# GLAD-RUC/DistEGNN

Hardware: NVIDIA H100
Metric: graph_steps_per_sec (higher is better)
Workload: dtype f32

## Files before the change

distegnn_b200/csrc/tc16.cuh:

```cuda
#pragma once
#include <cuda_fp16.h>

#include <type_traits>

#include "common.cuh"
#include "tile_mma.cuh"

namespace degnn {
namespace tc16 {

constexpr float RANGE = 3.0e4f;
__device__ __forceinline__ void split_pair(f32x2 x, uint32_t& hi, uint32_t& lo) {
    float x0, x1, l0, l1;
    upk2(x, x0, x1);
    const __half2 h = __floats2half2_rn(x0, x1);
    hi = *reinterpret_cast<const uint32_t*>(&h);
    const float2 hf = __half22float2(h);
    upk2(sub2(x, pk2(hf.x, hf.y)), l0, l1);
    const __half2 l = __floats2half2_rn(l0, l1);
    lo = *reinterpret_cast<const uint32_t*>(&l);
}

template <int NTHREADS>
__device__ __forceinline__ void stage_weight(__half* hi, __half* lo, const float* __restrict__ wt_kmajor, int n_off,
                                             int n_total, int tid, float scale = 1.0f) {
    static_assert((H * H) % NTHREADS == 0, "thread count must divide the matrix");
    constexpr int R = H * H / NTHREADS;
    const uint32_t lbo_h = (uint32_t)(n_total / 8) * 64u;
    float w[R];
#pragma unroll
    for (int r = 0; r < R; ++r) w[r] = __ldg(wt_kmajor + tid + r * NTHREADS);
#pragma unroll
    for (int r = 0; r < R; ++r) {
        const int i = tid + r * NTHREADS;
        const int k = i >> 6, n = (i & 63) + n_off;
        const float ws = w[r] * scale;
        const __half h = __float2half_rn(ws);
        const uint32_t o = (uint32_t)(k >> 3) * lbo_h + (uint32_t)(n >> 3) * 64u + (uint32_t)(n & 7) * 8u + (k & 7);
        hi[o] = h;
        lo[o] = __float2half_rn(ws - __half2float(h));
    }
}
__host__ __device__ constexpr uint32_t lbo_bytes(int n_total) { return (uint32_t)(n_total / 8) * 128u; }

template <uint32_t LBO>
__device__ __forceinline__ void mma_f16x3(uint32_t d, uint32_t a_hi, uint32_t a_lo, uint64_t b_hi, uint64_t b_lo,
                                          int nchunks, bool accumulate, int mb0, int nmb) {
    constexpr uint64_t B_KSTEP = (2 * LBO) >> 4, A_KSTEP = (2 * tmma::TM_COLGROUP_BYTES) >> 4, B_NCHUNK = (8 * 128) >> 4;
#pragma unroll 1
    for (int mb = mb0; mb < mb0 + nmb; ++mb) {
        const uint64_t ahi = tmma::make_desc(tmma::tm_addr_rc(64u * mb, a_hi), tmma::TM_COLGROUP_BYTES, 128);
        const uint64_t alo = tmma::make_desc(tmma::tm_addr_rc(64u * mb, a_lo), tmma::TM_COLGROUP_BYTES, 128);
#pragma unroll 1
        for (int nc = 0; nc < nchunks; ++nc) {
            float acc[32];
            if (accumulate) {
                tmma::frag_load(acc, d + 64u * nc, mb);
            } else {
#pragma unroll
                for (int i = 0; i < 32; ++i) acc[i] = 0.f;
            }
            const uint64_t bh = b_hi + nc * B_NCHUNK, bl = b_lo + nc * B_NCHUNK;
            tmma::wgmma_fence();
#pragma unroll
            for (int ks = 0; ks < 4; ++ks)
                tmma::wgmma_f16_m64n64k16(acc, alo + ks * A_KSTEP, bh + ks * B_KSTEP, (accumulate || ks > 0) ? 1u : 0u);
#pragma unroll
            for (int ks = 0; ks < 4; ++ks) tmma::wgmma_f16_m64n64k16(acc, ahi + ks * A_KSTEP, bl + ks * B_KSTEP, 1u);
#pragma unroll
            for (int ks = 0; ks < 4; ++ks) tmma::wgmma_f16_m64n64k16(acc, ahi + ks * A_KSTEP, bh + ks * B_KSTEP, 1u);
            tmma::wgmma_commit();
            tmma::wgmma_wait_all();
            tmma::frag_store(acc, d + 64u * nc, mb);
        }
    }
}

template <uint32_t LBO, bool ACCUMULATE = false>
__device__ __forceinline__ void mma_f16x3_rA(float (&d)[32], const uint32_t (&a_hi)[16], const uint32_t (&a_lo)[16],
                                             uint64_t b_hi, uint64_t b_lo) {
    constexpr uint64_t B_KSTEP = (2 * LBO) >> 4;
    auto mma = [&](auto acc, const uint32_t (&a)[16], int ks, uint64_t b) {
        tmma::wgmma_f16_m64n64k16_rA<decltype(acc)::value>(d, a[4 * ks], a[4 * ks + 1], a[4 * ks + 2], a[4 * ks + 3],
                                                            b + ks * B_KSTEP);
    };
    tmma::wgmma_fence();
    mma(std::integral_constant<bool, ACCUMULATE>{}, a_lo, 0, b_hi);
#pragma unroll
    for (int ks = 1; ks < 4; ++ks) mma(std::true_type{}, a_lo, ks, b_hi);
#pragma unroll
    for (int ks = 0; ks < 4; ++ks) mma(std::true_type{}, a_hi, ks, b_lo);
#pragma unroll
    for (int ks = 0; ks < 4; ++ks) mma(std::true_type{}, a_hi, ks, b_hi);
    tmma::wgmma_commit();
}
__device__ __forceinline__ void mma_f16x3_rA_wait(float (&d)[32], uint32_t (&a_hi)[16], uint32_t (&a_lo)[16]) {
    tmma::wgmma_wait_all();
#pragma unroll
    for (int i = 0; i < 32; ++i) tmma::wgmma_keep(d[i]);
#pragma unroll
    for (int i = 0; i < 16; ++i) {
        tmma::wgmma_keep(a_hi[i]);
        tmma::wgmma_keep(a_lo[i]);
    }
}

__device__ __forceinline__ bool row_overflow(__half2 mx) {
    return fmaxf(__low2float(mx), __high2float(mx)) > RANGE;
}
__device__ __forceinline__ void range_scale(float rowmax, float& s, float& inv_s) {
    const uint32_t eb = (__float_as_uint(rowmax) >> 23) & 0xffu;
    const uint32_t sb = eb > 141u ? 268u - eb : 127u;
    s = __uint_as_float((sb < 1u ? 1u : sb) << 23);
    inv_s = 1.0f / s;
}

constexpr std::false_type kFast{};
constexpr std::true_type kSafe{};
template <bool SCALED>
__device__ __forceinline__ void split16p(const f32x2 (&v)[8], float s, uint32_t (&hi)[8], uint32_t (&lo)[8],
                                         __half2& mx) {
#pragma unroll
    for (int j = 0; j < 8; ++j) {
        split_pair(SCALED ? mul2(v[j], bc2(s)) : v[j], hi[j], lo[j]);
        mx = __hmax2(mx, __habs2(*reinterpret_cast<const __half2*>(&hi[j])));
    }
}

}
}
```

distegnn_b200/csrc/tile_mma.cuh:

```cuda
#pragma once
#include <cuda_runtime.h>
#include <stdint.h>

namespace degnn {

extern __shared__ __align__(1024) uint8_t degnn_dyn_smem[];

namespace tmma {

constexpr uint32_t TM_COLGROUP_BYTES = 2048;
__host__ __device__ constexpr int tm_bytes(int ncols) { return ncols * 128 * 4; }

__device__ __forceinline__ uint32_t smem_u32(const void* p) {
    return (uint32_t)__cvta_generic_to_shared(p);
}

__device__ __forceinline__ uint32_t tm_addr_rc(uint32_t row, uint32_t col) {
    return smem_u32(degnn_dyn_smem) + (col >> 2) * TM_COLGROUP_BYTES + row * 16u + (col & 3u) * 4u;
}
__device__ __forceinline__ uint32_t tm_addr(uint32_t taddr) {
    return tm_addr_rc((taddr >> 16) + (threadIdx.x & 31u), taddr & 0xffffu);
}

__device__ __forceinline__ uint64_t make_desc(uint32_t smem_addr, uint32_t lbo, uint32_t sbo) {
    return (uint64_t)((smem_addr >> 4) & 0x3FFF) | ((uint64_t)((lbo >> 4) & 0x3FFF) << 16) |
           ((uint64_t)((sbo >> 4) & 0x3FFF) << 32);
}
__device__ __forceinline__ uint64_t make_b_desc(uint32_t smem_addr, uint32_t lbo, uint32_t sbo) {
    return make_desc(smem_addr, lbo, sbo);
}

__device__ __forceinline__ void fence_proxy_async_smem() { asm volatile("fence.proxy.async.shared::cta;" ::: "memory"); }
__device__ __forceinline__ void tm_st_fence() { fence_proxy_async_smem(); }

__device__ __forceinline__ void tm_st4(uint32_t taddr, const uint32_t (&r)[4]) {
    asm volatile("st.shared.v4.b32 [%0], {%1,%2,%3,%4};" ::"r"(tm_addr(taddr)), "r"(r[0]), "r"(r[1]), "r"(r[2]), "r"(r[3])
                 : "memory");
}
__device__ __forceinline__ void tm_ld4(uint32_t taddr, uint32_t* r) {
    asm volatile("ld.shared.v4.b32 {%0,%1,%2,%3}, [%4];" : "=r"(r[0]), "=r"(r[1]), "=r"(r[2]), "=r"(r[3]) : "r"(tm_addr(taddr))
                 : "memory");
}
__device__ __forceinline__ void tm_st8(uint32_t taddr, const uint32_t (&r)[8]) {
    tm_st4(taddr, *reinterpret_cast<const uint32_t(*)[4]>(&r[0]));
    tm_st4(taddr + 4, *reinterpret_cast<const uint32_t(*)[4]>(&r[4]));
}
__device__ __forceinline__ void tm_st16(uint32_t taddr, const uint32_t (&r)[16]) {
#pragma unroll
    for (int i = 0; i < 4; ++i) tm_st4(taddr + 4 * i, *reinterpret_cast<const uint32_t(*)[4]>(&r[4 * i]));
}
__device__ __forceinline__ void tm_ld8(uint32_t taddr, uint32_t (&r)[8]) {
    tm_ld4(taddr, &r[0]);
    tm_ld4(taddr + 4, &r[4]);
}
__device__ __forceinline__ void tm_ld16(uint32_t taddr, uint32_t (&r)[16]) {
#pragma unroll
    for (int i = 0; i < 4; ++i) tm_ld4(taddr + 4 * i, &r[4 * i]);
}
__device__ __forceinline__ void prefetch_l1(const void* p) { asm volatile("prefetch.global.L1 [%0];" ::"l"(p)); }
__device__ __forceinline__ void prefetch_l2(const void* p) { asm volatile("prefetch.global.L2 [%0];" ::"l"(p)); }

__device__ __forceinline__ void wgmma_fence() { asm volatile("wgmma.fence.sync.aligned;" ::: "memory"); }
__device__ __forceinline__ void wgmma_commit() { asm volatile("wgmma.commit_group.sync.aligned;" ::: "memory"); }
__device__ __forceinline__ void wgmma_wait_all() { asm volatile("wgmma.wait_group.sync.aligned 0;" ::: "memory"); }
__device__ __forceinline__ void wgmma_f16_m64n64k16(float (&d)[32], uint64_t a_desc, uint64_t b_desc, uint32_t accumulate) {
    asm volatile(
        "{\n\t"
        ".reg .pred p;\n\t"
        "setp.ne.b32 p, %34, 0;\n\t"
        "wgmma.mma_async.sync.aligned.m64n64k16.f32.f16.f16 "
        "{%0,%1,%2,%3,%4,%5,%6,%7,%8,%9,%10,%11,%12,%13,%14,%15,%16,%17,%18,%19,%20,%21,%22,%23,%24,%25,%26,%27,%28,%29,%30,%31},"
        " %32, %33, p, 1, 1, 0, 0;\n\t"
        "}\n"
        : "+f"(d[0]), "+f"(d[1]), "+f"(d[2]), "+f"(d[3]), "+f"(d[4]), "+f"(d[5]), "+f"(d[6]), "+f"(d[7]), "+f"(d[8]),
          "+f"(d[9]), "+f"(d[10]), "+f"(d[11]), "+f"(d[12]), "+f"(d[13]), "+f"(d[14]), "+f"(d[15]), "+f"(d[16]),
          "+f"(d[17]), "+f"(d[18]), "+f"(d[19]), "+f"(d[20]), "+f"(d[21]), "+f"(d[22]), "+f"(d[23]), "+f"(d[24]),
          "+f"(d[25]), "+f"(d[26]), "+f"(d[27]), "+f"(d[28]), "+f"(d[29]), "+f"(d[30]), "+f"(d[31])
        : "l"(a_desc), "l"(b_desc), "r"(accumulate)
        : "memory");
}
#define DEGNN_WGMMA_RA_D(c)                                                                                             \
    c(d[0]), c(d[1]), c(d[2]), c(d[3]), c(d[4]), c(d[5]), c(d[6]), c(d[7]), c(d[8]), c(d[9]), c(d[10]), c(d[11]),      \
        c(d[12]), c(d[13]), c(d[14]), c(d[15]), c(d[16]), c(d[17]), c(d[18]), c(d[19]), c(d[20]), c(d[21]), c(d[22]),  \
        c(d[23]), c(d[24]), c(d[25]), c(d[26]), c(d[27]), c(d[28]), c(d[29]), c(d[30]), c(d[31])
#define DEGNN_WGMMA_RA_ASM(scale_d)                                                                                     \
    "wgmma.mma_async.sync.aligned.m64n64k16.f32.f16.f16 "                                                               \
    "{%0,%1,%2,%3,%4,%5,%6,%7,%8,%9,%10,%11,%12,%13,%14,%15,%16,%17,%18,%19,%20,%21,%22,%23,%24,%25,%26,%27,%28,%29,%30," \
    "%31}, {%32,%33,%34,%35}, %36, " scale_d ", 1, 1, 0;\n"
template <bool ACCUMULATE>
__device__ __forceinline__ void wgmma_f16_m64n64k16_rA(float (&d)[32], uint32_t a0, uint32_t a1, uint32_t a2, uint32_t a3,
                                                       uint64_t b_desc) {
    if (ACCUMULATE)
        asm volatile(DEGNN_WGMMA_RA_ASM("1") : DEGNN_WGMMA_RA_D("+f")
                     : "r"(a0), "r"(a1), "r"(a2), "r"(a3), "l"(b_desc) : "memory");
    else
        asm volatile(DEGNN_WGMMA_RA_ASM("0") : DEGNN_WGMMA_RA_D("=f")
                     : "r"(a0), "r"(a1), "r"(a2), "r"(a3), "l"(b_desc) : "memory");
}
#undef DEGNN_WGMMA_RA_D
#undef DEGNN_WGMMA_RA_ASM
__device__ __forceinline__ void wgmma_keep(float& r) { asm volatile("" : "+f"(r)::"memory"); }
__device__ __forceinline__ void wgmma_keep(uint32_t& r) { asm volatile("" : "+r"(r)::"memory"); }
__device__ __forceinline__ void frag_rows(int mb, uint32_t& r0, uint32_t& q) {
    const uint32_t w = (threadIdx.x >> 5) & 3u, l = threadIdx.x & 31u;
    r0 = 64u * (uint32_t)mb + 16u * w + (l >> 2);
    q = l & 3u;
}
__device__ __forceinline__ void frag_store(const float (&d)[32], uint32_t col, int mb) {
    uint32_t r0, q;
    frag_rows(mb, r0, q);
#pragma unroll
    for (int j = 0; j < 8; ++j) {
        const uint32_t c = col + 8u * j + 2u * q;
        const uint32_t a0 = tm_addr_rc(r0, c), a1 = tm_addr_rc(r0 + 8u, c);
        asm volatile("st.shared.v2.f32 [%0], {%1,%2};" ::"r"(a0), "f"(d[4 * j]), "f"(d[4 * j + 1]) : "memory");
        asm volatile("st.shared.v2.f32 [%0], {%1,%2};" ::"r"(a1), "f"(d[4 * j + 2]), "f"(d[4 * j + 3]) : "memory");
    }
}
__device__ __forceinline__ void frag_load(float (&d)[32], uint32_t col, int mb) {
    uint32_t r0, q;
    frag_rows(mb, r0, q);
#pragma unroll
    for (int j = 0; j < 8; ++j) {
        const uint32_t c = col + 8u * j + 2u * q;
        asm volatile("ld.shared.v2.f32 {%0,%1}, [%2];" : "=f"(d[4 * j]), "=f"(d[4 * j + 1]) : "r"(tm_addr_rc(r0, c)) : "memory");
        asm volatile("ld.shared.v2.f32 {%0,%1}, [%2];" : "=f"(d[4 * j + 2]), "=f"(d[4 * j + 3]) : "r"(tm_addr_rc(r0 + 8u, c))
                     : "memory");
    }
}

__device__ __forceinline__ void mbar_init(uint64_t* bar, uint32_t count) {
    asm volatile("mbarrier.init.shared::cta.b64 [%0], %1;" ::"r"(smem_u32(bar)), "r"(count) : "memory");
}
__device__ __forceinline__ void fence_mbar_init() { asm volatile("fence.mbarrier_init.release.cluster;" ::: "memory"); }
__device__ __forceinline__ void mbar_expect_tx(uint64_t* bar, uint32_t bytes) {
    asm volatile("mbarrier.arrive.expect_tx.shared::cta.b64 _, [%0], %1;" ::"r"(smem_u32(bar)), "r"(bytes) : "memory");
}
__device__ __forceinline__ void mbar_wait(uint64_t* bar, uint32_t parity) {
    asm volatile(
        "{\n\t"
        ".reg .pred p;\n\t"
        "WAIT_LOOP:\n\t"
        "mbarrier.try_wait.parity.shared::cta.b64 p, [%0], %1;\n\t"
        "@p bra WAIT_DONE;\n\t"
        "bra WAIT_LOOP;\n\t"
        "WAIT_DONE:\n\t"
        "}\n" ::"r"(smem_u32(bar)),
        "r"(parity)
        : "memory");
}

__device__ __forceinline__ void bulk_g2s(void* smem_dst, const void* gsrc, uint32_t bytes, uint64_t* bar) {
    asm volatile("cp.async.bulk.shared::cluster.global.mbarrier::complete_tx::bytes [%0], [%1], %2, [%3];" ::"r"(
                     smem_u32(smem_dst)),
                 "l"(gsrc), "r"(bytes), "r"(smem_u32(bar))
                 : "memory");
}

__device__ __forceinline__ void cp_async16(void* smem_dst, const void* gsrc) {
    asm volatile("cp.async.cg.shared.global [%0], [%1], 16;" ::"r"(smem_u32(smem_dst)), "l"(gsrc) : "memory");
}
__device__ __forceinline__ void cp_async8(void* smem_dst, const void* gsrc) {
    asm volatile("cp.async.ca.shared.global [%0], [%1], 8;" ::"r"(smem_u32(smem_dst)), "l"(gsrc) : "memory");
}
__device__ __forceinline__ void cp_async4(void* smem_dst, const void* gsrc) {
    asm volatile("cp.async.ca.shared.global [%0], [%1], 4;" ::"r"(smem_u32(smem_dst)), "l"(gsrc) : "memory");
}
__device__ __forceinline__ void cp_async_commit() { asm volatile("cp.async.commit_group;" ::: "memory"); }
__device__ __forceinline__ void cp_async_wait_all() { asm volatile("cp.async.wait_group 0;" ::: "memory"); }
__device__ __forceinline__ void red_add_v2(float* gdst, float a, float b) {
    asm volatile("red.global.add.v2.f32 [%0], {%1, %2};" ::"l"(gdst), "f"(a), "f"(b) : "memory");
}

__device__ __forceinline__ void named_bar(uint32_t id, uint32_t nthreads) {
    asm volatile("bar.sync %0, %1;" ::"r"(id), "r"(nthreads) : "memory");
}

}
}
```

distegnn_b200/csrc/virtual_layer_tc16.cu:

```cuda
#include "common.cuh"
#include "det.cuh"
#include "tc16.cuh"
#include "tile_mma.cuh"

namespace degnn {

struct VirtT16Args {
    int64_t N;
    int B, C;
    unsigned flags;
    const int32_t* batch;
    const float* x4;
    const float* Hn;
    const float* Xv;
    const float* G;
    const float* w1r;
    const float* w2; const float* b2;
    const float* wxv; const float* bxv; const float* w3xv;
    const float* wx; const float* bx; const float* w3x;
    float* agg_v;
    float* trans_v;
    float* vsum;
    float* slots;
    int chunk_shift;
};

constexpr int VW_WG = 4;
constexpr int VW_THREADS = 128 * VW_WG, VW_WARPS = VW_THREADS / 32;
constexpr int VW_TILE = 64;
constexpr int VW_ROW = 72;
constexpr int VW_W = 64 * 64;
constexpr uint32_t VW_LBO = 1024;
__host__ __device__ constexpr int vw_smem_floats(int C) {
    return 6 * VW_W / 2 + 6 * H + VW_WARPS * 16 * VW_ROW + VW_WG * VW_TILE * 6 + VW_WG * C * VW_ROW + VW_WARPS * C * H
           + VW_WARPS * 4 * C;
}
__host__ __device__ constexpr int vw_smem_bytes(int C) { return vw_smem_floats(C) * 4; }
using tc16::kFast;
using tc16::kSafe;

static_assert(VW_TILE == DET_VTILE, "det.cuh sizes the slots from the tile");
template <bool DET>
__global__ void __launch_bounds__(VW_THREADS, 1) virtual_layer_t16_kernel(const VirtT16Args a) {
    using namespace tmma;
    const int C = a.C;
    __half* W2hi = reinterpret_cast<__half*>(degnn_dyn_smem);
    __half* W2lo = W2hi + VW_W;
    __half* Wxvhi = W2lo + VW_W;
    __half* Wxvlo = Wxvhi + VW_W;
    __half* Wxhi = Wxvlo + VW_W;
    __half* Wxlo = Wxhi + VW_W;
    float* w1rs = reinterpret_cast<float*>(Wxlo + VW_W);
    float* b2s = w1rs + H;
    float* bxvs = b2s + H;
    float* w3xvs = bxvs + H;
    float* bxs = w3xvs + H;
    float* w3xs = bxs + H;
    float* stage_all = w3xs + H;
    float* dX_all = stage_all + VW_WARPS * 16 * VW_ROW;
    float* phi_all = dX_all + VW_WG * VW_TILE * 4;
    float* gs_all = phi_all + VW_WG * VW_TILE * 2;
    float* accH_all = gs_all + VW_WG * C * VW_ROW;
    float* accX_all = accH_all + VW_WARPS * C * H;

    const int tid = threadIdx.x;
    const int lane = tid & 31;
    const int warp = tid >> 5;
    const int wg = warp >> 2;
    const int w = warp & 3;
    const int t = tid & 127;
    const int g = lane >> 2, q = lane & 3;
    const int K = 4 + 3 * C + H * C;
    const bool need_feat = !(a.flags & DISTEGNN_FLAG_LAST);
    const int TN = VW_TILE / C;
    const bool warp_local = (16 % C) == 0;

    tc16::stage_weight<VW_THREADS>(W2hi, W2lo, a.w2, 0, 64, tid, SILU_T_IN);
    tc16::stage_weight<VW_THREADS>(Wxvhi, Wxvlo, a.wxv, 0, 64, tid);
    tc16::stage_weight<VW_THREADS>(Wxhi, Wxlo, a.wx, 0, 64, tid);
    if (tid < H) {
        w1rs[tid] = a.w1r[tid];
        b2s[tid] = a.b2[tid] * SILU_T_IN;
        bxvs[tid] = a.bxv[tid] * SILU_T_IN;
        w3xvs[tid] = a.w3xv[tid] * SILU_T_OUT;
        bxs[tid] = a.bx[tid] * SILU_T_IN;
        w3xs[tid] = a.w3x[tid] * SILU_T_OUT;
    }
    for (int i = tid; i < VW_WARPS * (C * H + 4 * C); i += VW_THREADS) accH_all[i] = 0.f;
    fence_proxy_async_smem();
    __syncthreads();

    const uint64_t bW0 = make_b_desc(smem_u32(W2hi), VW_LBO, 128);
    auto bW = [&](int k) { return bW0 + (uint64_t)(k * (VW_W * 2 / 16)); };
    float* tile_s = stage_all + wg * VW_TILE * VW_ROW;
    float* dXs = dX_all + wg * VW_TILE * 4;
    float* phis = phi_all + wg * VW_TILE * 2;
    float* gs = gs_all + wg * C * VW_ROW;
    float* accH = accH_all + warp * C * H;
    float* accX = accX_all + warp * 4 * C;
    float* accH_g = accH_all + 4 * wg * C * H;
    float* accX_g = accX_all + 4 * wg * 4 * C;
    const uint32_t bar_id = 1 + wg;
    int cur_graph = -1;

    auto flush = [&](int gr) {
        if (gr < 0) return;
        float* dst = a.vsum + (size_t)gr * K;
        if (need_feat)
            for (int i = t; i < C * H; i += 128) {
                float s = 0.f;
#pragma unroll
                for (int k = 0; k < 4; ++k) {
                    s += accH_g[k * C * H + i];
                    accH_g[k * C * H + i] = 0.f;
                }
                atomicAdd(dst + 4 + 3 * C + i, s * SILU_T_OUT);
            }
        if (t < 3 * C) {
            float s = 0.f;
#pragma unroll
            for (int k = 0; k < 4; ++k) {
                s += accX_g[k * 4 * C + t];
                accX_g[k * 4 * C + t] = 0.f;
            }
            atomicAdd(dst + 4 + t, s);
        }
    };

    const int num_tiles = (int)((a.N + TN - 1) / TN);
    const int stride = (int)gridDim.x * VW_WG;
    const int CH = 1 << a.chunk_shift;
    auto next_tile = [&](int tl) {
        if constexpr (DET) return (tl + 1) % CH != 0 ? tl + 1 : tl + 1 + (stride - 1) * CH;
        else return tl + stride;
    };
    float* accG = accH_all + 4 * wg * C * H;
    float* accXG = accX_all + 4 * wg * 4 * C;
    int curM = -1, curX = -1, cont = -1;
    auto det_dst = [&](int gr, int tl) {
        return gr == cont ? a.slots + (size_t)(tl >> a.chunk_shift) * K : a.vsum + (size_t)gr * K;
    };
    auto det_flush_m = [&](int tl) {
        for (int c = t >> 5; c < C; c += 4) {
            f32x2* acc = reinterpret_cast<f32x2*>(accG + c * H + 2 * (t & 31));
            if (curM >= 0) {
                float* dst = det_dst(curM, tl) + 4 + 3 * C + c * H + 2 * (t & 31);
                upk2(mul2(*acc, bc2(SILU_T_OUT)), dst[0], dst[1]);
            }
            *acc = 0ull;
        }
    };
    auto det_flush_x = [&](int tl) {
        if (t < 3 * C) {
            if (curX >= 0) det_dst(curX, tl)[4 + t] = accXG[t];
            accXG[t] = 0.f;
        }
    };
    const int ra = 16 * w + g, rb = ra + 8;
    const float* colp = tile_s + 2 * lane;

    for (int tile = DET ? ((int)blockIdx.x * VW_WG + wg) * CH : (int)blockIdx.x * VW_WG + wg; tile < num_tiles;
         tile = next_tile(tile)) {
        const int64_t n0 = (int64_t)tile * TN;
        if (DET && tile % CH == 0)
            cont = (n0 > 0 && __ldg(a.batch + n0 - 1) == __ldg(a.batch + n0)) ? __ldg(a.batch + n0) : -1;
        const int nvalid = (int)min((int64_t)TN, a.N - n0);
        const int rows = nvalid * C;
        {
            const int64_t nn0 = (int64_t)next_tile(tile) * TN;
            const int nnv = (int)min((int64_t)TN, a.N - nn0);
            for (int i = t; i < 2 * nnv; i += 128) prefetch_l1(a.Hn + (size_t)nn0 * H + 32 * i);
            if (nnv > 0) {
                if (t < (nnv * 16 + 127) / 128) prefetch_l1(a.x4 + (size_t)nn0 * 4 + 32 * t);
                if (t == 127) prefetch_l1(a.batch + nn0);
                if (t == 126) prefetch_l1(a.batch + nn0 + nnv - 1);
            }
        }
        const int g_first = __ldg(a.batch + n0), g_last = __ldg(a.batch + n0 + nvalid - 1);
        const bool single = (g_first == g_last);
        if (single && g_first != cur_graph) {
            named_bar(bar_id, 128);
            if constexpr (!DET) flush(cur_graph);
            cur_graph = g_first;
            for (int i = t; i < C * (H / 4); i += 128) {
                const int c = i / (H / 4), q4 = i - c * (H / 4);
                *reinterpret_cast<float4*>(gs + c * VW_ROW + 4 * q4) = ldg4(a.G + ((size_t)g_first * C + c) * H + 4 * q4);
            }
            named_bar(bar_id, 128);
        }

        const bool va = ra < rows, vb = rb < rows;
        const float* pa;
        const float* pb;
        const float* ga;
        const float* gb;
        float vra, vrb;
        {
            auto row_geo = [&](int r, bool v, const float*& hrow, const float*& grow) {
                const int nl = v ? r / C : 0, ch = v ? r - nl * C : 0;
                const size_t node = (size_t)(n0 + nl);
                const int gr = single ? g_first : __ldg(a.batch + node);
                const float4 xi = ldg4(a.x4 + node * 4);
                const float* Xg = a.Xv + (size_t)gr * 3 * C;
                const float dx = __ldg(Xg + ch) - xi.x, dy = __ldg(Xg + C + ch) - xi.y, dz = __ldg(Xg + 2 * C + ch) - xi.z;
                if (q == 0) *reinterpret_cast<float4*>(dXs + 4 * r) = make_float4(dx, dy, dz, 0.f);
                hrow = a.Hn + node * H + 2 * q;
                grow = (gr == cur_graph ? (const float*)(gs + ch * VW_ROW) : a.G + ((size_t)gr * C + ch) * H) + 2 * q;
                return sqrtf(dx * dx + dy * dy + dz * dz);
            };
            vra = row_geo(ra, va, pa, ga);
            vrb = row_geo(rb, vb, pb, gb);
        }
        auto pre = [&](int j, const float* hrow, const float* grow, float vr) {
            const f32x2 hh = __ldg(reinterpret_cast<const f32x2*>(hrow + 8 * j));
            const f32x2 gg = *reinterpret_cast<const f32x2*>(grow + 8 * j);
            return fma2(bc2(vr), *reinterpret_cast<const f32x2*>(w1rs + 8 * j + 2 * q), add2(hh, gg));
        };
        uint32_t ahi[16], alo[16];
        float inv1a = 1.0f, inv1b = 1.0f;
        {
            __half2 mx = __floats2half2_rn(0.f, 0.f);
            float qmax = 0.f;
#pragma unroll
            for (int j = 0; j < 8; ++j) {
                f32x2 xa = pre(j, pa, ga, vra), xb = pre(j, pb, gb, vrb);
                silu4p<false>(xa, xb, qmax);
                if (!va) xa = 0ull;
                if (!vb) xb = 0ull;
                tc16::split_pair(xa, ahi[2 * j], alo[2 * j]);
                tc16::split_pair(xb, ahi[2 * j + 1], alo[2 * j + 1]);
                mx = __hmax2(mx, __hmax2(*reinterpret_cast<const __half2*>(&ahi[2 * j]),
                                         *reinterpret_cast<const __half2*>(&ahi[2 * j + 1])));
            }
            if (__any_sync(FULL, tc16::row_overflow(mx) || silu_q_overflow(qmax))) {
                float fa = 0.f, fb = 0.f, sa, sb;
#pragma unroll 1
                for (int j = 0; j < 8; ++j) {
                    f32x2 xa = pre(j, pa, ga, vra), xb = pre(j, pb, gb, vrb);
                    silu4p<true>(xa, xb, qmax);
                    float v0, v1;
                    upk2(xa, v0, v1);
                    if (va) fa = fmaxf(fa, fmaxf(v0, v1));
                    upk2(xb, v0, v1);
                    if (vb) fb = fmaxf(fb, fmaxf(v0, v1));
                }
                fa = fmaxf(fa, __shfl_xor_sync(FULL, fa, 1));
                fa = fmaxf(fa, __shfl_xor_sync(FULL, fa, 2));
                fb = fmaxf(fb, __shfl_xor_sync(FULL, fb, 1));
                fb = fmaxf(fb, __shfl_xor_sync(FULL, fb, 2));
                tc16::range_scale(fa, sa, inv1a);
                tc16::range_scale(fb, sb, inv1b);
#pragma unroll
                for (int j = 0; j < 8; ++j) {
                    f32x2 xa = pre(j, pa, ga, vra), xb = pre(j, pb, gb, vrb);
                    silu4p<true>(xa, xb, qmax);
                    if (!va) xa = 0ull;
                    if (!vb) xb = 0ull;
                    tc16::split_pair(mul2(xa, bc2(sa)), ahi[2 * j], alo[2 * j]);
                    tc16::split_pair(mul2(xb, bc2(sb)), ahi[2 * j + 1], alo[2 * j + 1]);
                }
            }
        }

        float d[32];
        tc16::mma_f16x3_rA<VW_LBO>(d, ahi, alo, bW(0), bW(1));
        tc16::mma_f16x3_rA_wait(d, ahi, alo);

        float inv2a = 1.0f, inv2b = 1.0f, s2a = 1.0f, s2b = 1.0f;
        auto m_pair = [&](int j, f32x2& ma, f32x2& mb) {
            const f32x2 bb = *reinterpret_cast<const f32x2*>(b2s + 8 * j + 2 * q);
            ma = fma2(pk2(d[4 * j + 0], d[4 * j + 1]), bc2(inv1a), bb);
            mb = fma2(pk2(d[4 * j + 2], d[4 * j + 3]), bc2(inv1b), bb);
        };
        auto store_m = [&](int j, f32x2 ma, f32x2 mb) {
            *reinterpret_cast<f32x2*>(tile_s + ra * VW_ROW + 8 * j + 2 * q) = ma;
            *reinterpret_cast<f32x2*>(tile_s + rb * VW_ROW + 8 * j + 2 * q) = mb;
        };
        {
            __half2 mx = __floats2half2_rn(0.f, 0.f);
            float qmax = 0.f;
#pragma unroll
            for (int j = 0; j < 8; ++j) {
                f32x2 ma, mb;
                m_pair(j, ma, mb);
                silu4t<false>(ma, mb, qmax);
                store_m(j, ma, mb);
                tc16::split_pair(ma, ahi[2 * j], alo[2 * j]);
                tc16::split_pair(mb, ahi[2 * j + 1], alo[2 * j + 1]);
                mx = __hmin2(mx, __hmin2(*reinterpret_cast<const __half2*>(&ahi[2 * j]),
                                         *reinterpret_cast<const __half2*>(&ahi[2 * j + 1])));
            }
            if (__any_sync(FULL, fminf(__low2float(mx), __high2float(mx)) < -tc16::RANGE || silu_q_overflow(qmax))) {
                float fa = 0.f, fb = 0.f;
#pragma unroll
                for (int j = 0; j < 8; ++j) {
                    f32x2 ma, mb;
                    m_pair(j, ma, mb);
                    silu4t<true>(ma, mb, qmax);
                    store_m(j, ma, mb);
                    float v0, v1;
                    upk2(ma, v0, v1);
                    fa = fmaxf(fa, -fminf(v0, v1));
                    upk2(mb, v0, v1);
                    fb = fmaxf(fb, -fminf(v0, v1));
                }
                fa = fmaxf(fa, __shfl_xor_sync(FULL, fa, 1));
                fa = fmaxf(fa, __shfl_xor_sync(FULL, fa, 2));
                fb = fmaxf(fb, __shfl_xor_sync(FULL, fb, 1));
                fb = fmaxf(fb, __shfl_xor_sync(FULL, fb, 2));
                tc16::range_scale(fa, s2a, inv2a);
                tc16::range_scale(fb, s2b, inv2b);
#pragma unroll
                for (int j = 0; j < 8; ++j) {
                    f32x2 ma, mb;
                    m_pair(j, ma, mb);
                    silu4t<true>(ma, mb, qmax);
                    tc16::split_pair(mul2(ma, bc2(s2a)), ahi[2 * j], alo[2 * j]);
                    tc16::split_pair(mul2(mb, bc2(s2b)), ahi[2 * j + 1], alo[2 * j + 1]);
                }
            }
        }

        const int nb = warp_local ? (16 * w) / C : w;
        const int ne = warp_local ? min(nb + 16 / C, nvalid) : nvalid;
        const int ns = warp_local ? 1 : 4;
        const int r_end = min(16 * w + 16, rows);

        tc16::mma_f16x3_rA<VW_LBO>(d, ahi, alo, bW(2), bW(3));
        if (need_feat) {
            if (warp_local && !DET) __syncwarp();
            else named_bar(bar_id, 128);
            auto ld2 = [](const float* p) { return *reinterpret_cast<const f32x2*>(p); };
            const f32x2 invC2 = bc2(SILU_T_OUT / (float)C);
#pragma unroll 1
            for (int n = nb; n < ne; n += ns) {
                const float* base = colp + (n * C) * VW_ROW;
                f32x2 s0 = 0ull, s1 = 0ull;
                int c = 0;
#pragma unroll 1
                for (; c + 1 < C; c += 2) {
                    s0 = add2(s0, ld2(base + c * VW_ROW));
                    s1 = add2(s1, ld2(base + (c + 1) * VW_ROW));
                }
                if (c < C) s0 = add2(s0, ld2(base + c * VW_ROW));
                *reinterpret_cast<f32x2*>(a.agg_v + (size_t)(n0 + n) * H + 2 * lane) = mul2(add2(s0, s1), invC2);
            }
            if constexpr (DET) {
                for (int n = 0; n < nvalid; ++n) {
                    const int gr = single ? g_first : __ldg(a.batch + n0 + n);
                    if (gr != curM) {
                        det_flush_m(tile);
                        curM = gr;
                    }
                    for (int c = t >> 5; c < C; c += 4) {
                        f32x2* acc = reinterpret_cast<f32x2*>(accG + c * H + 2 * (t & 31));
                        *acc = add2(*acc, ld2(tile_s + (n * C + c) * VW_ROW + 2 * (t & 31)));
                    }
                }
            } else if (single) {
                const int cn = min(C, 16);
#pragma unroll 1
                for (int i = 0; i < cn; ++i) {
                    const int r = 16 * w + i;
                    if (r >= r_end) break;
                    f32x2 s = ld2(colp + r * VW_ROW);
#pragma unroll 1
                    for (int r2 = r + C; r2 < r_end; r2 += C) s = add2(s, ld2(colp + r2 * VW_ROW));
                    f32x2* acc = reinterpret_cast<f32x2*>(accH + (r % C) * H + 2 * lane);
                    *acc = add2(*acc, s);
                }
            } else {
#pragma unroll 1
                for (int r = 16 * w; r < r_end; ++r) {
                    const int n = r / C, c = r - n * C;
                    float* dst = a.vsum + (size_t)__ldg(a.batch + n0 + n) * K + 4 + 3 * C + c * H + 2 * lane;
                    float v0, v1;
                    upk2(ld2(colp + r * VW_ROW), v0, v1);
                    atomicAdd(dst, v0 * SILU_T_OUT);
                    atomicAdd(dst + 1, v1 * SILU_T_OUT);
                }
            }
        }
        tc16::mma_f16x3_rA_wait(d, ahi, alo);

        auto head = [&](const float* bs, const float* ws, float& phia, float& phib) {
#pragma unroll
            for (int j = 0; j < 8; ++j) {
                const f32x2 bb = *reinterpret_cast<const f32x2*>(bs + 8 * j + 2 * q);
                upk2(fma2(pk2(d[4 * j + 0], d[4 * j + 1]), bc2(inv2a), bb), d[4 * j + 0], d[4 * j + 1]);
                upk2(fma2(pk2(d[4 * j + 2], d[4 * j + 3]), bc2(inv2b), bb), d[4 * j + 2], d[4 * j + 3]);
            }
            float qmax = 0.f;
            f32x2 pha, phb;
            auto pass = [&](auto safe) {
                pha = phb = bc2(0.f);
#pragma unroll
                for (int j = 0; j < 8; ++j) {
                    const f32x2 ww = *reinterpret_cast<const f32x2*>(ws + 8 * j + 2 * q);
                    f32x2 sa = pk2(d[4 * j + 0], d[4 * j + 1]), sb = pk2(d[4 * j + 2], d[4 * j + 3]);
                    silu4t<decltype(safe)::value>(sa, sb, qmax);
                    pha = fma2(sa, ww, pha);
                    phb = fma2(sb, ww, phb);
                }
            };
            pass(kFast);
            if (__any_sync(FULL, silu_q_overflow(qmax))) pass(kSafe);
            float p0, p1;
            upk2(pha, p0, p1);
            phia = p0 + p1;
            upk2(phb, p0, p1);
            phib = p0 + p1;
            phia += __shfl_xor_sync(FULL, phia, 1);
            phia += __shfl_xor_sync(FULL, phia, 2);
            phib += __shfl_xor_sync(FULL, phib, 1);
            phib += __shfl_xor_sync(FULL, phib, 2);
        };
        {
            float phia, phib;
            head(bxvs, w3xvs, phia, phib);
            if (q == 0) {
                phis[ra] = phia;
                phis[rb] = phib;
            }
        }

#pragma unroll
        for (int j = 0; j < 8; ++j) {
            const f32x2 ma = *reinterpret_cast<const f32x2*>(tile_s + ra * VW_ROW + 8 * j + 2 * q);
            const f32x2 mb = *reinterpret_cast<const f32x2*>(tile_s + rb * VW_ROW + 8 * j + 2 * q);
            tc16::split_pair(mul2(ma, bc2(s2a)), ahi[2 * j], alo[2 * j]);
            tc16::split_pair(mul2(mb, bc2(s2b)), ahi[2 * j + 1], alo[2 * j + 1]);
        }
        tc16::mma_f16x3_rA<VW_LBO>(d, ahi, alo, bW(4), bW(5));
        if (warp_local) __syncwarp();
        else named_bar(bar_id, 128);
        for (int i = lane; i < (ne - nb + ns - 1) / ns * 3; i += 32) {
            const int n = nb + (i / 3) * ns, dd = i - 3 * (i / 3);
            float s = 0.f;
            for (int c = 0; c < C; ++c) s = fmaf(-dXs[4 * (n * C + c) + dd], phis[n * C + c], s);
            a.trans_v[(size_t)(n0 + n) * 4 + dd] = s / (float)C;
        }
        tc16::mma_f16x3_rA_wait(d, ahi, alo);

        {
            float phia, phib;
            head(bxs, w3xs, phia, phib);
            if (q == 0) {
                phis[VW_TILE + ra] = phia;
                phis[VW_TILE + rb] = phib;
            }
        }
        __syncwarp();
        const float* phx = phis + VW_TILE;
        if constexpr (DET) {
            named_bar(bar_id, 128);
            if (t < 3 * C) {
                const int dd = t / C, c = t - dd * C;
                for (int n = 0; n < nvalid; ++n) {
                    const int gr = single ? g_first : __ldg(a.batch + n0 + n);
                    if (gr != curX) {
                        det_flush_x(tile);
                        curX = gr;
                    }
                    accXG[t] = fmaf(dXs[4 * (n * C + c) + dd], phx[n * C + c], accXG[t]);
                }
            }
        } else if (single) {
            const int cn = min(C, 16);
            for (int it = lane; it < 3 * cn; it += 32) {
                const int dd = it / cn, r = 16 * w + (it - dd * cn);
                if (r < r_end) {
                    float s = 0.f;
                    for (int r2 = r; r2 < r_end; r2 += C) s = fmaf(dXs[4 * r2 + dd], phx[r2], s);
                    accX[dd * C + r % C] += s;
                }
            }
        } else {
            for (int it = lane; it < 48; it += 32) {
                const int r = 16 * w + it / 3, dd = it - 3 * (it / 3);
                if (r < r_end) {
                    const int n = r / C, c = r - n * C;
                    atomicAdd(a.vsum + (size_t)__ldg(a.batch + n0 + n) * K + 4 + dd * C + c, dXs[4 * r + dd] * phx[r]);
                }
            }
        }
        if (warp_local && !DET) __syncwarp();
        else named_bar(bar_id, 128);
        if (DET && ((tile + 1) % CH == 0 || tile + 1 >= num_tiles)) {
            if (need_feat) det_flush_m(tile);
            det_flush_x(tile);
            curM = curX = -1;
        }
    }
    if constexpr (!DET) {
        named_bar(bar_id, 128);
        flush(cur_graph);
    }
}

}

namespace degnn {

template <bool DET>
static int virtual_layer_fwd(int64_t n_nodes, int n_graphs, int A, int C, int Na, unsigned flags, const int32_t* batch32,
                             const float* x4, const float* Hn, const float* Xv, const float* G, const float* layer_params,
                             float* agg_v, float* trans_v, float* vsum, void* workspace, int64_t workspace_bytes,
                             void* stream, int max_ctas) {
    if (int rc = check_dims(A, C, Na)) return rc;
    if (n_nodes == 0) return DISTEGNN_OK;
    DEGNN_CHECK_ARG(n_nodes > 0 && n_graphs > 0, "bad size");
    DEGNN_CHECK_ARG(batch32 && x4 && Hn && Xv && G && layer_params && trans_v && vsum, "null pointer");
    DEGNN_CHECK_ARG((flags & DISTEGNN_FLAG_LAST) || agg_v, "null agg_v");
    if (DET)
        if (int rc = det_check_workspace(n_nodes, -1, C, workspace, workspace_bytes, "distegnn_virtual_layer_fwd_det"))
            return rc;
    Layout L = make_layout(A, C, Na);
    VirtT16Args a;
    a.N = n_nodes; a.B = n_graphs; a.C = C; a.flags = flags;
    a.batch = batch32; a.x4 = x4; a.Hn = Hn; a.Xv = Xv; a.G = G;
    a.w1r = layer_params + L.off[DISTEGNN_P_V_W1R];
    a.w2 = layer_params + L.off[DISTEGNN_P_V_W2];
    a.b2 = layer_params + L.off[DISTEGNN_P_V_B2];
    a.wxv = layer_params + L.off[DISTEGNN_P_V_WXV];
    a.bxv = layer_params + L.off[DISTEGNN_P_V_BXV];
    a.w3xv = layer_params + L.off[DISTEGNN_P_V_W3XV];
    a.wx = layer_params + L.off[DISTEGNN_P_V_WX];
    a.bx = layer_params + L.off[DISTEGNN_P_V_BX];
    a.w3x = layer_params + L.off[DISTEGNN_P_V_W3X];
    a.agg_v = agg_v; a.trans_v = trans_v; a.vsum = vsum;
    a.slots = DET ? det_vsum_slots(workspace) : nullptr;
    a.chunk_shift = DET ? det_chunk_shift(n_nodes, C) : 0;
    static_assert(vw_smem_bytes(DISTEGNN_MAX_CHANNELS) <= 232448, "the widest C must fit");
    ensure_dynamic_smem((const void*)virtual_layer_t16_kernel<DET>, vw_smem_bytes(DISTEGNN_MAX_CHANNELS));
    const int TN = VW_TILE / C;
    const int64_t tiles = (n_nodes + TN - 1) / TN;
    const int64_t units = DET ? det_chunks(n_nodes, C) : tiles;
    DEGNN_CHECK_ARG(tiles + ((int64_t)sm_count() * VW_WG << (DET ? det_chunk_shift(n_nodes, C) : 0)) < ((int64_t)1 << 31),
                    "too many nodes");
    int64_t grid = (units + VW_WG - 1) / VW_WG;
    if (grid > sm_count()) grid = sm_count();
    if (DET) grid = det_grid(grid, max_ctas);
    virtual_layer_t16_kernel<DET><<<(unsigned)grid, VW_THREADS, vw_smem_bytes(C), (cudaStream_t)stream>>>(a);
    DEGNN_CHECK_LAUNCH();
    return DISTEGNN_OK;
}

int virtual_layer_fwd_det(int64_t n_nodes, int n_graphs, int A, int C, int Na, unsigned flags, const int32_t* batch32,
                          const float* x4, const float* Hn, const float* Xv, const float* G, const float* layer_params,
                          float* agg_v, float* trans_v, float* vsum, void* workspace, int64_t workspace_bytes,
                          void* stream, int max_ctas) {
    return virtual_layer_fwd<true>(n_nodes, n_graphs, A, C, Na, flags, batch32, x4, Hn, Xv, G, layer_params, agg_v,
                                   trans_v, vsum, workspace, workspace_bytes, stream, max_ctas);
}

}

extern "C" int distegnn_virtual_layer_fwd(int64_t n_nodes, int n_graphs, int A, int C, int Na, unsigned flags,
                                          const int32_t* batch32, const float* x4, const float* Hn,
                                          const float* Xv, const float* G, const float* layer_params,
                                          float* agg_v, float* trans_v, float* vsum, void* stream) {
    return degnn::virtual_layer_fwd<false>(n_nodes, n_graphs, A, C, Na, flags, batch32, x4, Hn, Xv, G, layer_params,
                                           agg_v, trans_v, vsum, nullptr, 0, stream, 0);
}

extern "C" int distegnn_virtual_layer_fwd_det(int64_t n_nodes, int n_graphs, int A, int C, int Na, unsigned flags,
                                              const int32_t* batch32, const float* x4, const float* Hn,
                                              const float* Xv, const float* G, const float* layer_params,
                                              float* agg_v, float* trans_v, float* vsum, void* workspace,
                                              int64_t workspace_bytes, void* stream) {
    return degnn::virtual_layer_fwd_det(n_nodes, n_graphs, A, C, Na, flags, batch32, x4, Hn, Xv, G, layer_params,
                                        agg_v, trans_v, vsum, workspace, workspace_bytes, stream, 0);
}
```

Before: 33.25.

## Fuse the two head GEMMs into one m64n128 wgmma with shared safe-path recompute

Stages the wxv and wx head weights side by side as a single 128-wide B operand and issues one m64n128k16 wgmma sequence instead of two back-to-back m64n64 sequences. Both heads' SiLU passes then run on the 64-register accumulator. The rare overflow path now needs the A fragments again, so it re-splits them and recomputes under a block-level OR barrier. This removes one MMA issue/wait round and a sync, at the cost of 32 more live accumulator registers per thread and a possible full recompute when either head overflows.

```diff
diff --git a/distegnn_b200/csrc/tc16.cuh b/distegnn_b200/csrc/tc16.cuh
--- a/distegnn_b200/csrc/tc16.cuh
+++ b/distegnn_b200/csrc/tc16.cuh
@@ -76,13 +76,13 @@
     }
 }
 
-template <uint32_t LBO, bool ACCUMULATE = false>
-__device__ __forceinline__ void mma_f16x3_rA(float (&d)[32], const uint32_t (&a_hi)[16], const uint32_t (&a_lo)[16],
+template <uint32_t LBO, bool ACCUMULATE = false, int ND>
+__device__ __forceinline__ void mma_f16x3_rA(float (&d)[ND], const uint32_t (&a_hi)[16], const uint32_t (&a_lo)[16],
                                              uint64_t b_hi, uint64_t b_lo) {
     constexpr uint64_t B_KSTEP = (2 * LBO) >> 4;
     auto mma = [&](auto acc, const uint32_t (&a)[16], int ks, uint64_t b) {
-        tmma::wgmma_f16_m64n64k16_rA<decltype(acc)::value>(d, a[4 * ks], a[4 * ks + 1], a[4 * ks + 2], a[4 * ks + 3],
-                                                            b + ks * B_KSTEP);
+        tmma::wgmma_f16_rA<decltype(acc)::value>(d, a[4 * ks], a[4 * ks + 1], a[4 * ks + 2], a[4 * ks + 3],
+                                                 b + ks * B_KSTEP);
     };
     tmma::wgmma_fence();
     mma(std::integral_constant<bool, ACCUMULATE>{}, a_lo, 0, b_hi);
@@ -94,10 +94,11 @@
     for (int ks = 0; ks < 4; ++ks) mma(std::true_type{}, a_hi, ks, b_hi);
     tmma::wgmma_commit();
 }
-__device__ __forceinline__ void mma_f16x3_rA_wait(float (&d)[32], uint32_t (&a_hi)[16], uint32_t (&a_lo)[16]) {
+template <int ND>
+__device__ __forceinline__ void mma_f16x3_rA_wait(float (&d)[ND], uint32_t (&a_hi)[16], uint32_t (&a_lo)[16]) {
     tmma::wgmma_wait_all();
 #pragma unroll
-    for (int i = 0; i < 32; ++i) tmma::wgmma_keep(d[i]);
+    for (int i = 0; i < ND; ++i) tmma::wgmma_keep(d[i]);
 #pragma unroll
     for (int i = 0; i < 16; ++i) {
         tmma::wgmma_keep(a_hi[i]);
diff --git a/distegnn_b200/csrc/tile_mma.cuh b/distegnn_b200/csrc/tile_mma.cuh
--- a/distegnn_b200/csrc/tile_mma.cuh
+++ b/distegnn_b200/csrc/tile_mma.cuh
@@ -99,6 +99,38 @@
 }
 #undef DEGNN_WGMMA_RA_D
 #undef DEGNN_WGMMA_RA_ASM
+#define DEGNN_WGMMA_D8(c, b) c(d[b]), c(d[b + 1]), c(d[b + 2]), c(d[b + 3]), c(d[b + 4]), c(d[b + 5]), c(d[b + 6]), c(d[b + 7])
+#define DEGNN_WGMMA_RA128_D(c)                                                                                          \
+    DEGNN_WGMMA_D8(c, 0), DEGNN_WGMMA_D8(c, 8), DEGNN_WGMMA_D8(c, 16), DEGNN_WGMMA_D8(c, 24), DEGNN_WGMMA_D8(c, 32),    \
+        DEGNN_WGMMA_D8(c, 40), DEGNN_WGMMA_D8(c, 48), DEGNN_WGMMA_D8(c, 56)
+#define DEGNN_WGMMA_RA128_ASM(scale_d)                                                                                  \
+    "wgmma.mma_async.sync.aligned.m64n128k16.f32.f16.f16 "                                                              \
+    "{%0,%1,%2,%3,%4,%5,%6,%7,%8,%9,%10,%11,%12,%13,%14,%15,%16,%17,%18,%19,%20,%21,%22,%23,%24,%25,%26,%27,%28,%29,%30," \
+    "%31,%32,%33,%34,%35,%36,%37,%38,%39,%40,%41,%42,%43,%44,%45,%46,%47,%48,%49,%50,%51,%52,%53,%54,%55,%56,%57,%58,"   \
+    "%59,%60,%61,%62,%63}, {%64,%65,%66,%67}, %68, " scale_d ", 1, 1, 0;\n"
+template <bool ACCUMULATE>
+__device__ __forceinline__ void wgmma_f16_m64n128k16_rA(float (&d)[64], uint32_t a0, uint32_t a1, uint32_t a2,
+                                                        uint32_t a3, uint64_t b_desc) {
+    if (ACCUMULATE)
+        asm volatile(DEGNN_WGMMA_RA128_ASM("1") : DEGNN_WGMMA_RA128_D("+f")
+                     : "r"(a0), "r"(a1), "r"(a2), "r"(a3), "l"(b_desc) : "memory");
+    else
+        asm volatile(DEGNN_WGMMA_RA128_ASM("0") : DEGNN_WGMMA_RA128_D("=f")
+                     : "r"(a0), "r"(a1), "r"(a2), "r"(a3), "l"(b_desc) : "memory");
+}
+#undef DEGNN_WGMMA_D8
+#undef DEGNN_WGMMA_RA128_D
+#undef DEGNN_WGMMA_RA128_ASM
+template <bool ACCUMULATE>
+__device__ __forceinline__ void wgmma_f16_rA(float (&d)[32], uint32_t a0, uint32_t a1, uint32_t a2, uint32_t a3,
+                                             uint64_t b_desc) {
+    wgmma_f16_m64n64k16_rA<ACCUMULATE>(d, a0, a1, a2, a3, b_desc);
+}
+template <bool ACCUMULATE>
+__device__ __forceinline__ void wgmma_f16_rA(float (&d)[64], uint32_t a0, uint32_t a1, uint32_t a2, uint32_t a3,
+                                             uint64_t b_desc) {
+    wgmma_f16_m64n128k16_rA<ACCUMULATE>(d, a0, a1, a2, a3, b_desc);
+}
 __device__ __forceinline__ void wgmma_keep(float& r) { asm volatile("" : "+f"(r)::"memory"); }
 __device__ __forceinline__ void wgmma_keep(uint32_t& r) { asm volatile("" : "+r"(r)::"memory"); }
 __device__ __forceinline__ void frag_rows(int mb, uint32_t& r0, uint32_t& q) {
@@ -175,6 +207,13 @@
 __device__ __forceinline__ void named_bar(uint32_t id, uint32_t nthreads) {
     asm volatile("bar.sync %0, %1;" ::"r"(id), "r"(nthreads) : "memory");
 }
-
-}
-}
+__device__ __forceinline__ bool named_bar_or(uint32_t id, uint32_t nthreads, bool pred) {
+    uint32_t r;
+    asm volatile(
+        "{\n\t.reg .pred p, q;\n\tsetp.ne.u32 p, %1, 0;\n\tbar.red.or.pred q, %2, %3, p;\n\tselp.u32 %0, 1, 0, q;\n\t}"
+        : "=r"(r) : "r"((uint32_t)pred), "r"(id), "r"(nthreads) : "memory");
+    return r != 0;
+}
+
+}
+}
diff --git a/distegnn_b200/csrc/virtual_layer_tc16.cu b/distegnn_b200/csrc/virtual_layer_tc16.cu
--- a/distegnn_b200/csrc/virtual_layer_tc16.cu
+++ b/distegnn_b200/csrc/virtual_layer_tc16.cu
@@ -31,6 +31,7 @@
 constexpr int VW_ROW = 72;
 constexpr int VW_W = 64 * 64;
 constexpr uint32_t VW_LBO = 1024;
+constexpr uint32_t VW_LBO_HEADS = 2048;
 __host__ __device__ constexpr int vw_smem_floats(int C) {
     return 6 * VW_W / 2 + 6 * H + VW_WARPS * 16 * VW_ROW + VW_WG * VW_TILE * 6 + VW_WG * C * VW_ROW + VW_WARPS * C * H
            + VW_WARPS * 4 * C;
@@ -46,11 +47,9 @@
     const int C = a.C;
     __half* W2hi = reinterpret_cast<__half*>(degnn_dyn_smem);
     __half* W2lo = W2hi + VW_W;
-    __half* Wxvhi = W2lo + VW_W;
-    __half* Wxvlo = Wxvhi + VW_W;
-    __half* Wxhi = Wxvlo + VW_W;
-    __half* Wxlo = Wxhi + VW_W;
-    float* w1rs = reinterpret_cast<float*>(Wxlo + VW_W);
+    __half* Whhi = W2lo + VW_W;
+    __half* Whlo = Whhi + 2 * VW_W;
+    float* w1rs = reinterpret_cast<float*>(Whlo + 2 * VW_W);
     float* b2s = w1rs + H;
     float* bxvs = b2s + H;
     float* w3xvs = bxvs + H;
@@ -76,8 +75,8 @@
     const bool warp_local = (16 % C) == 0;
 
     tc16::stage_weight<VW_THREADS>(W2hi, W2lo, a.w2, 0, 64, tid, SILU_T_IN);
-    tc16::stage_weight<VW_THREADS>(Wxvhi, Wxvlo, a.wxv, 0, 64, tid);
-    tc16::stage_weight<VW_THREADS>(Wxhi, Wxlo, a.wx, 0, 64, tid);
+    tc16::stage_weight<VW_THREADS>(Whhi, Whlo, a.wxv, 0, 128, tid);
+    tc16::stage_weight<VW_THREADS>(Whhi, Whlo, a.wx, 64, 128, tid);
     if (tid < H) {
         w1rs[tid] = a.w1r[tid];
         b2s[tid] = a.b2[tid] * SILU_T_IN;
@@ -90,8 +89,9 @@
     fence_proxy_async_smem();
     __syncthreads();
 
-    const uint64_t bW0 = make_b_desc(smem_u32(W2hi), VW_LBO, 128);
-    auto bW = [&](int k) { return bW0 + (uint64_t)(k * (VW_W * 2 / 16)); };
+    const uint64_t bW2 = make_b_desc(smem_u32(W2hi), VW_LBO, 128);
+    const uint64_t bWh = make_b_desc(smem_u32(Whhi), VW_LBO_HEADS, 128);
+    constexpr uint64_t W2_LO = VW_W * 2 / 16, WH_LO = 2 * VW_W * 2 / 16;
     float* tile_s = stage_all + wg * VW_TILE * VW_ROW;
     float* dXs = dX_all + wg * VW_TILE * 4;
     float* phis = phi_all + wg * VW_TILE * 2;
@@ -263,7 +263,7 @@
         }
 
         float d[32];
-        tc16::mma_f16x3_rA<VW_LBO>(d, ahi, alo, bW(0), bW(1));
+        tc16::mma_f16x3_rA<VW_LBO>(d, ahi, alo, bW2, bW2 + W2_LO);
         tc16::mma_f16x3_rA_wait(d, ahi, alo);
 
         float inv2a = 1.0f, inv2b = 1.0f, s2a = 1.0f, s2b = 1.0f;
@@ -326,7 +326,8 @@
         const int ns = warp_local ? 1 : 4;
         const int r_end = min(16 * w + 16, rows);
 
-        tc16::mma_f16x3_rA<VW_LBO>(d, ahi, alo, bW(2), bW(3));
+        float dh[64];
+        tc16::mma_f16x3_rA<VW_LBO_HEADS>(dh, ahi, alo, bWh, bWh + WH_LO);
         if (need_feat) {
             if (warp_local && !DET) __syncwarp();
             else named_bar(bar_id, 128);
@@ -381,58 +382,60 @@
                 }
             }
         }
-        tc16::mma_f16x3_rA_wait(d, ahi, alo);
-
-        auto head = [&](const float* bs, const float* ws, float& phia, float& phib) {
+        tc16::mma_f16x3_rA_wait(dh, ahi, alo);
+
+        f32x2 pha[2], phb[2];
+        float qmax[2] = {0.f, 0.f};
+        auto pass = [&](auto safe, int h) {
+            const float* bs = h ? bxs : bxvs;
+            const float* ws = h ? w3xs : w3xvs;
+            pha[h] = phb[h] = bc2(0.f);
 #pragma unroll
             for (int j = 0; j < 8; ++j) {
+                const float* d = dh + 32 * h + 4 * j;
                 const f32x2 bb = *reinterpret_cast<const f32x2*>(bs + 8 * j + 2 * q);
-                upk2(fma2(pk2(d[4 * j + 0], d[4 * j + 1]), bc2(inv2a), bb), d[4 * j + 0], d[4 * j + 1]);
-                upk2(fma2(pk2(d[4 * j + 2], d[4 * j + 3]), bc2(inv2b), bb), d[4 * j + 2], d[4 * j + 3]);
-            }
-            float qmax = 0.f;
-            f32x2 pha, phb;
-            auto pass = [&](auto safe) {
-                pha = phb = bc2(0.f);
-#pragma unroll
-                for (int j = 0; j < 8; ++j) {
-                    const f32x2 ww = *reinterpret_cast<const f32x2*>(ws + 8 * j + 2 * q);
-                    f32x2 sa = pk2(d[4 * j + 0], d[4 * j + 1]), sb = pk2(d[4 * j + 2], d[4 * j + 3]);
-                    silu4t<decltype(safe)::value>(sa, sb, qmax);
-                    pha = fma2(sa, ww, pha);
-                    phb = fma2(sb, ww, phb);
-                }
-            };
-            pass(kFast);
-            if (__any_sync(FULL, silu_q_overflow(qmax))) pass(kSafe);
+                const f32x2 ww = *reinterpret_cast<const f32x2*>(ws + 8 * j + 2 * q);
+                f32x2 sa = fma2(pk2(d[0], d[1]), bc2(inv2a), bb), sb = fma2(pk2(d[2], d[3]), bc2(inv2b), bb);
+                silu4t<decltype(safe)::value>(sa, sb, qmax[h]);
+                pha[h] = fma2(sa, ww, pha[h]);
+                phb[h] = fma2(sb, ww, phb[h]);
+            }
+        };
+        pass(kFast, 0);
+        pass(kFast, 1);
+        const bool cold0 = __any_sync(FULL, silu_q_overflow(qmax[0]));
+        const bool cold1 = __any_sync(FULL, silu_q_overflow(qmax[1]));
+        if (named_bar_or(bar_id, 128, cold0 || cold1)) {
+#pragma unroll
+            for (int j = 0; j < 8; ++j) {
+                const f32x2 ma = *reinterpret_cast<const f32x2*>(tile_s + ra * VW_ROW + 8 * j + 2 * q);
+                const f32x2 mb = *reinterpret_cast<const f32x2*>(tile_s + rb * VW_ROW + 8 * j + 2 * q);
+                tc16::split_pair(mul2(ma, bc2(s2a)), ahi[2 * j], alo[2 * j]);
+                tc16::split_pair(mul2(mb, bc2(s2b)), ahi[2 * j + 1], alo[2 * j + 1]);
+            }
+            tc16::mma_f16x3_rA<VW_LBO_HEADS>(dh, ahi, alo, bWh, bWh + WH_LO);
+            tc16::mma_f16x3_rA_wait(dh, ahi, alo);
+            if (cold0) pass(kSafe, 0);
+            if (cold1) pass(kSafe, 1);
+        }
+#pragma unroll
+        for (int h = 0; h < 2; ++h) {
             float p0, p1;
-            upk2(pha, p0, p1);
-            phia = p0 + p1;
-            upk2(phb, p0, p1);
-            phib = p0 + p1;
+            upk2(pha[h], p0, p1);
+            float phia = p0 + p1;
+            upk2(phb[h], p0, p1);
+            float phib = p0 + p1;
             phia += __shfl_xor_sync(FULL, phia, 1);
             phia += __shfl_xor_sync(FULL, phia, 2);
             phib += __shfl_xor_sync(FULL, phib, 1);
             phib += __shfl_xor_sync(FULL, phib, 2);
-        };
-        {
-            float phia, phib;
-            head(bxvs, w3xvs, phia, phib);
             if (q == 0) {
-                phis[ra] = phia;
-                phis[rb] = phib;
-            }
-        }
-
-#pragma unroll
-        for (int j = 0; j < 8; ++j) {
-            const f32x2 ma = *reinterpret_cast<const f32x2*>(tile_s + ra * VW_ROW + 8 * j + 2 * q);
-            const f32x2 mb = *reinterpret_cast<const f32x2*>(tile_s + rb * VW_ROW + 8 * j + 2 * q);
-            tc16::split_pair(mul2(ma, bc2(s2a)), ahi[2 * j], alo[2 * j]);
-            tc16::split_pair(mul2(mb, bc2(s2b)), ahi[2 * j + 1], alo[2 * j + 1]);
-        }
-        tc16::mma_f16x3_rA<VW_LBO>(d, ahi, alo, bW(4), bW(5));
-        if (warp_local) __syncwarp();
+                phis[VW_TILE * h + ra] = phia;
+                phis[VW_TILE * h + rb] = phib;
+            }
+        }
+
+        if (warp_local && !DET) __syncwarp();
         else named_bar(bar_id, 128);
         for (int i = lane; i < (ne - nb + ns - 1) / ns * 3; i += 32) {
             const int n = nb + (i / 3) * ns, dd = i - 3 * (i / 3);
@@ -440,20 +443,8 @@
             for (int c = 0; c < C; ++c) s = fmaf(-dXs[4 * (n * C + c) + dd], phis[n * C + c], s);
             a.trans_v[(size_t)(n0 + n) * 4 + dd] = s / (float)C;
         }
-        tc16::mma_f16x3_rA_wait(d, ahi, alo);
-
-        {
-            float phia, phib;
-            head(bxs, w3xs, phia, phib);
-            if (q == 0) {
-                phis[VW_TILE + ra] = phia;
-                phis[VW_TILE + rb] = phib;
-            }
-        }
-        __syncwarp();
         const float* phx = phis + VW_TILE;
         if constexpr (DET) {
-            named_bar(bar_id, 128);
             if (t < 3 * C) {
                 const int dd = t / C, c = t - dd * C;
                 for (int n = 0; n < nvalid; ++n) {
```

Result: faster. 33.93, median of 6 (+2.0%).
